# zer0int/OpenVision

Measured on AMD Instinct MI355X. Metric: images/sec (node) ViT-L/14@224 fwd+InfoNCE, higher is better.
Workload: dtype bf16; 1 GPU; vit-large-patch14-224: image tower + text tower (T=80) + InfoNCE, per-GPU batch 256, formula weights, bf16 MFMA / fp32 accumulate; fp8_mask=0, global_batch=256, micro_batches=1, parallelism=dp1

## Files before the change

openvision_amd/csrc/attention.hip:

```cpp
#include "common.h"
#include <stdlib.h>

namespace {

struct AttnArgs {
    const ov_bf16* qkv; int64_t ldq;
    ov_bf16* out; int64_t ldo;
    int B, L, H, nqt, KC;
    float scale_log2;
    int prefix;
};

typedef __attribute__((address_space(3))) s16x4_t* lds_s16x4_ptr;
typedef const __attribute__((address_space(1))) void* gptr_t;
typedef __attribute__((address_space(3))) void* lptr_t;

__device__ __forceinline__ bf16x8_t tr_pair(const char* p0, const char* p1) {
    const s16x4_t a = __builtin_amdgcn_ds_read_tr16_b64_v4i16((lds_s16x4_ptr)p0);
    const s16x4_t b = __builtin_amdgcn_ds_read_tr16_b64_v4i16((lds_s16x4_ptr)p1);
    typedef short s16x8_t __attribute__((ext_vector_type(8)));
    const s16x8_t c = {a[0], a[1], a[2], a[3], b[0], b[1], b[2], b[3]};
    return __builtin_bit_cast(bf16x8_t, c);
}

__device__ __forceinline__ u32x2_t tr_read_asm(const char* p) {
    u32x2_t v;
    const unsigned addr = (unsigned)(uintptr_t)(__attribute__((address_space(3))) const char*)p;
    asm volatile("ds_read_b64_tr_b16 %0, %1" : "=v"(v) : "v"(addr));
    return v;
}
__device__ __forceinline__ void tr_wait(u32x2_t (&t)[8]) {
    asm volatile("s_waitcnt lgkmcnt(0)"
                 : "+v"(t[0]), "+v"(t[1]), "+v"(t[2]), "+v"(t[3]), "+v"(t[4]), "+v"(t[5]), "+v"(t[6]), "+v"(t[7]));
}
__device__ __forceinline__ bf16x8_t tr_join(u32x2_t a, u32x2_t b) {
    const u32x4_t w = {a[0], a[1], b[0], b[1]};
    return __builtin_bit_cast(bf16x8_t, w);
}

__device__ __forceinline__ unsigned pack_fp8x4(float a, float b, float c, float d) {
    int w = 0;
    w = __builtin_amdgcn_cvt_pk_fp8_f32(__builtin_amdgcn_fmed3f(a, -448.f, 448.f), __builtin_amdgcn_fmed3f(b, -448.f, 448.f), w, false);
    w = __builtin_amdgcn_cvt_pk_fp8_f32(__builtin_amdgcn_fmed3f(c, -448.f, 448.f), __builtin_amdgcn_fmed3f(d, -448.f, 448.f), w, true);
    return (unsigned)w;
}

struct AttnPArgs {
    const ov_bf16* qkv; int64_t ldq;
    ov_bf16* out; int64_t ldo;
    int L, H, nqt, KC, nheads;
    float scale_log2;
    const float* out_amax;
    float* amax_next;
    int lone_valu;
    float* lse;
};

__device__ __forceinline__ void stage_head(const AttnPArgs& a, int bh, char* slot, int wave, int lane, int nthreads) {
    const int b = bh / a.H, h = bh - b * a.H;
    const int HD = a.H * 64, KC = a.KC, L = a.L;
    const char* base = (const char*)(a.qkv + (int64_t)b * L * a.ldq + h * 64);
    const unsigned rowb = (unsigned)(a.ldq * 2);
    const unsigned last = (unsigned)(L - 1) * rowb;
    char* ks = slot;
    char* vs = slot + KC * 128;
    const int nchunk = KC * 8;
    for (int q0c = wave * 64; q0c < nchunk; q0c += nthreads) {
        {
            const int kkey = (q0c + lane) >> 3;
            const unsigned ro = kkey < L ? (unsigned)kkey * rowb : last;
            const int c = (lane & 7) ^ ((kkey >> 1) & 7);
            __builtin_amdgcn_global_load_lds((gptr_t)(base + (ro + (unsigned)((HD + c * 8) * 2))), (lptr_t)(ks + q0c * 16), 16, 0, 0);
        }
        {
            const int dh = q0c >= KC * 4 ? 1 : 0;
            const int vkey = (q0c - dh * KC * 4 + lane) >> 2;
            const unsigned ro = vkey < L ? (unsigned)vkey * rowb : last;
            __builtin_amdgcn_global_load_lds((gptr_t)(base + (ro + (unsigned)((2 * HD + (dh * 4 + (lane & 3)) * 8) * 2))),
                                             (lptr_t)(vs + q0c * 16), 16, 0, 0);
        }
    }
}

__device__ __forceinline__ float max3_asm(float x, float y, float z) {
    float d;
    asm("v_max3_f32 %0, %1, %2, %3" : "=v"(d) : "v"(x), "v"(y), "v"(z));
    return d;
}
typedef float f32x2_t __attribute__((ext_vector_type(2)));
__device__ __forceinline__ void exp_rows(f32x16_t& s, float c, float nm, f32x2_t& acc) {
    const f32x2_t cc = {c, c}, mm = {nm, nm};
#pragma unroll
    for (int i = 0; i < 8; ++i) {
        f32x2_t v = {s[2 * i], s[2 * i + 1]};
        v = __builtin_elementwise_fma(v, cc, mm);
        v[0] = __builtin_amdgcn_exp2f(v[0]);
        v[1] = __builtin_amdgcn_exp2f(v[1]);
        acc += v;
        s[2 * i] = v[0];
        s[2 * i + 1] = v[1];
    }
}
template <int OFF>
__device__ __forceinline__ u32x2_t tr_read_off(unsigned addr) {
    u32x2_t v;
    asm volatile("ds_read_b64_tr_b16 %0, %1 offset:%2" : "=v"(v) : "v"(addr), "n"(OFF));
    return v;
}

template <bool DEEP, bool OUT8, bool LSE = false>
__global__ __launch_bounds__(DEEP ? 512 : 640, DEEP ? 2 : 3) void attn_fwd_hd64_persist(const AttnPArgs a) {
    extern __shared__ __attribute__((aligned(16))) char smem[];
    const int tid = threadIdx.x;
    const int lane = tid & 63;
    const int wave = __builtin_amdgcn_readfirstlane(tid >> 6);
    const int r = lane & 31, h2 = lane >> 5;
    const int L = a.L, KC = a.KC;
    const int slot_bytes = KC * 256;
    const int nk_tiles = (L + 31) >> 5;
    const bool lone_on = a.lone_valu != 0;
    const bool lone_key = lone_on && (L & 31) == 1 && (nk_tiles & 1) && nk_tiles > 1;
    const int n = (a.nheads - (int)blockIdx.x + (int)gridDim.x - 1) / (int)gridDim.x;
    if (n <= 0) return;
    const float inv8 = OUT8 ? __uint_as_float(__builtin_amdgcn_readfirstlane(__float_as_uint(448.0f / (2.0f * fmaxf(*a.out_amax, 1e-30f))))) : 1.0f;
    const float next_thr = (OUT8 && a.amax_next != nullptr)
                               ? __uint_as_float(__builtin_amdgcn_readfirstlane(__float_as_uint(*a.amax_next))) : 0.f;

    const int kb = r * 128 + ((h2 ^ ((r >> 1) & 7)) << 4);
    const int vi = lane & 15, vg = (lane >> 4) & 1;
    const int v_lane0 = KC * 128 + (4 * h2 + (vi >> 2)) * 64 + (16 * vg + 4 * (vi & 3)) * 2;
    const int v_lane1 = v_lane0 + KC * 64;
    const int q0 = wave * 32;
    int qrow = q0 + r;
    qrow = qrow < L ? qrow : L - 1;

    auto head_base = [&](int bh) {
        const int b = bh / a.H, h = bh - b * a.H;
        return a.qkv + (int64_t)b * L * a.ldq + h * 64;
    };
    auto row_offset = [&](int ld, int per_h2, unsigned bytes) {
        unsigned lf = (unsigned)lane;
        asm volatile("" : "+v"(lf));
        int qr = q0 + (int)(lf & 31u);
        qr = qr < L ? qr : L - 1;
        return (unsigned)(qr * ld + per_h2 * (int)(lf >> 5)) * bytes;
    };
    auto load_q = [&](u32x4_t (&q)[4], int bh) {
        const ov_bf16* qb = head_base(bh);
        const unsigned qoff = row_offset((int)a.ldq, 8, 2u);
        asm volatile("global_load_dwordx4 %0, %1, %2" : "=v"(q[0]) : "v"(qoff), "s"(qb) : "memory");
        asm volatile("global_load_dwordx4 %0, %1, %2 offset:32" : "=v"(q[1]) : "v"(qoff), "s"(qb) : "memory");
        asm volatile("global_load_dwordx4 %0, %1, %2 offset:64" : "=v"(q[2]) : "v"(qoff), "s"(qb) : "memory");
        asm volatile("global_load_dwordx4 %0, %1, %2 offset:96" : "=v"(q[3]) : "v"(qoff), "s"(qb) : "memory");
    };
    stage_head(a, blockIdx.x, smem, wave, lane, blockDim.x);
    u32x4_t qn[4];
    load_q(qn, blockIdx.x);
    asm volatile("s_waitcnt vmcnt(0)" : "+v"(qn[0]), "+v"(qn[1]), "+v"(qn[2]), "+v"(qn[3]) :: "memory");

    for (int j = 0; j < n; ++j) {
        const int bh = blockIdx.x + j * gridDim.x;
        bf16x8_t qf[4];
#pragma unroll
        for (int st = 0; st < 4; ++st) qf[st] = __builtin_bit_cast(bf16x8_t, qn[st]);
        asm volatile("s_barrier" ::: "memory");
        if (j + 1 < n) stage_head(a, bh + gridDim.x, smem + ((j + 1) & 1) * slot_bytes, wave, lane, blockDim.x);
        const char* ks = smem + (j & 1) * slot_bytes;
        const unsigned ks_u = (unsigned)(uintptr_t)(__attribute__((address_space(3))) const char*)ks;

        float m = -INFINITY, lsum = 0.f;
        f32x16_t o0, o1;
#pragma unroll
        for (int i = 0; i < 16; ++i) { o0[i] = 0.f; o1[i] = 0.f; }
        bf16x8_t kfa[4], kfb[4];
        auto load_k = [&](bf16x8_t (&kf)[4], int kt) {
            const unsigned kp = (unsigned)(kt * 4096 + kb);
#pragma unroll
            for (int st = 0; st < 4; ++st) kf[st] = *(const bf16x8_t*)(ks + (kp ^ (unsigned)(st * 32)));
        };
        auto mask_tail = [&](f32x16_t& sc, int kt) {
            if (kt * 32 + 32 > L) {
#pragma unroll
                for (int i = 0; i < 16; ++i) {
                    const int key = kt * 32 + (i & 3) + 8 * (i >> 2) + 4 * h2;
                    if (key >= L) sc[i] = -INFINITY;
                }
            }
        };
        auto tile_max = [&](const f32x16_t& sc) {
            float mx = max3_asm(max3_asm(sc[0], sc[1], sc[2]), max3_asm(sc[3], sc[4], sc[5]), max3_asm(sc[6], sc[7], sc[8]));
            return max3_asm(mx, max3_asm(sc[9], sc[10], sc[11]), max3_asm(max3_asm(sc[12], sc[13], sc[14]), sc[15], sc[15]));
        };
        auto pack_p = [&](const f32x16_t& sc, int st) {
            const u32x4_t w = {pack_bf16x2(sc[8 * st + 0], sc[8 * st + 1]), pack_bf16x2(sc[8 * st + 2], sc[8 * st + 3]),
                               pack_bf16x2(sc[8 * st + 4], sc[8 * st + 5]), pack_bf16x2(sc[8 * st + 6], sc[8 * st + 7])};
            return __builtin_bit_cast(bf16x8_t, w);
        };
        const int npair = nk_tiles >> 1;
        load_k(kfa, 0);
        if (DEEP && npair > 0) load_k(kfb, 1);
        for (int it = 0; it < npair; ++it) {
            const int kt = 2 * it;
            const unsigned va0 = ks_u + kt * 2048 + v_lane0, va1 = ks_u + kt * 2048 + v_lane1;
            if (!DEEP) load_k(kfb, kt + 1);
            u32x2_t vt[8], vu[8];
            auto read_vt = [&]() {
                vt[0] = tr_read_off<0>(va0);    vt[1] = tr_read_off<512>(va0);
                vt[2] = tr_read_off<0>(va1);    vt[3] = tr_read_off<512>(va1);
                vt[4] = tr_read_off<1024>(va0); vt[5] = tr_read_off<1536>(va0);
                vt[6] = tr_read_off<1024>(va1); vt[7] = tr_read_off<1536>(va1);
            };
            if (DEEP) read_vt();
            if (DEEP) {
                vu[0] = tr_read_off<2048>(va0); vu[1] = tr_read_off<2560>(va0);
                vu[2] = tr_read_off<2048>(va1); vu[3] = tr_read_off<2560>(va1);
                vu[4] = tr_read_off<3072>(va0); vu[5] = tr_read_off<3584>(va0);
                vu[6] = tr_read_off<3072>(va1); vu[7] = tr_read_off<3584>(va1);
            }
            f32x16_t sa, sb;
#pragma unroll
            for (int i = 0; i < 16; ++i) { sa[i] = 0.f; sb[i] = 0.f; }
#pragma unroll
            for (int st = 0; st < 4; ++st) sa = __builtin_amdgcn_mfma_f32_32x32x16_bf16(kfa[st], qf[st], sa, 0, 0, 0);
#pragma unroll
            for (int st = 0; st < 4; ++st) sb = __builtin_amdgcn_mfma_f32_32x32x16_bf16(kfb[st], qf[st], sb, 0, 0, 0);
            if (!DEEP) read_vt();
            if (kt + 2 < nk_tiles) load_k(kfa, kt + 2);
            else if (DEEP) asm volatile("s_nop 7" : "+v"(sb));
            if (DEEP && kt + 3 < nk_tiles) load_k(kfb, kt + 3);
            mask_tail(sb, kt + 1);
            float mx = fmaxf(tile_max(sa), tile_max(sb));
            {
                const auto sw = __builtin_amdgcn_permlane32_swap(__float_as_uint(mx), __float_as_uint(mx), false, false);
                mx = fmaxf(__uint_as_float(sw[0]), __uint_as_float(sw[1])) * a.scale_log2;
            }
            if (!__all(mx - m <= 8.0f)) {
                const float mn = fmaxf(m, mx);
                const float alpha = __builtin_amdgcn_exp2f(m - mn);
                m = mn;
                lsum *= alpha;
#pragma unroll
                for (int i = 0; i < 16; ++i) { o0[i] *= alpha; o1[i] *= alpha; }
            }
            const float nm = -m;
            f32x2_t ps = {0.f, 0.f};
            exp_rows(sa, a.scale_log2, nm, ps);
            exp_rows(sb, a.scale_log2, nm, ps);
            lsum += ps[0] + ps[1];
            const bf16x8_t pa0 = pack_p(sa, 0), pa1 = pack_p(sa, 1), pb0 = pack_p(sb, 0), pb1 = pack_p(sb, 1);
            tr_wait(vt);
            __builtin_amdgcn_sched_barrier(0);
            if (!DEEP) {
                vu[0] = tr_read_off<2048>(va0); vu[1] = tr_read_off<2560>(va0);
                vu[2] = tr_read_off<2048>(va1); vu[3] = tr_read_off<2560>(va1);
                vu[4] = tr_read_off<3072>(va0); vu[5] = tr_read_off<3584>(va0);
                vu[6] = tr_read_off<3072>(va1); vu[7] = tr_read_off<3584>(va1);
            }
            o0 = __builtin_amdgcn_mfma_f32_32x32x16_bf16(tr_join(vt[0], vt[1]), pa0, o0, 0, 0, 0);
            o1 = __builtin_amdgcn_mfma_f32_32x32x16_bf16(tr_join(vt[2], vt[3]), pa0, o1, 0, 0, 0);
            o0 = __builtin_amdgcn_mfma_f32_32x32x16_bf16(tr_join(vt[4], vt[5]), pa1, o0, 0, 0, 0);
            o1 = __builtin_amdgcn_mfma_f32_32x32x16_bf16(tr_join(vt[6], vt[7]), pa1, o1, 0, 0, 0);
            tr_wait(vu);
            __builtin_amdgcn_sched_barrier(0);
            o0 = __builtin_amdgcn_mfma_f32_32x32x16_bf16(tr_join(vu[0], vu[1]), pb0, o0, 0, 0, 0);
            o1 = __builtin_amdgcn_mfma_f32_32x32x16_bf16(tr_join(vu[2], vu[3]), pb0, o1, 0, 0, 0);
            o0 = __builtin_amdgcn_mfma_f32_32x32x16_bf16(tr_join(vu[4], vu[5]), pb1, o0, 0, 0, 0);
            o1 = __builtin_amdgcn_mfma_f32_32x32x16_bf16(tr_join(vu[6], vu[7]), pb1, o1, 0, 0, 0);
        }
        if (j + 1 < n) load_q(qn, bh + gridDim.x);
        if (lone_key) {
            float s0 = 0.f, s1 = 0.f;
#pragma unroll
            for (int st = 0; st < 4; ++st) {
                const u32x4_t kq = __builtin_bit_cast(u32x4_t, kfa[st]), qq = __builtin_bit_cast(u32x4_t, qf[st]);
                asm("v_dot2c_f32_bf16 %0, %1, %2" : "+v"(s0) : "v"(qq[0]), "v"(kq[0]));
                asm("v_dot2c_f32_bf16 %0, %1, %2" : "+v"(s1) : "v"(qq[1]), "v"(kq[1]));
                asm("v_dot2c_f32_bf16 %0, %1, %2" : "+v"(s0) : "v"(qq[2]), "v"(kq[2]));
                asm("v_dot2c_f32_bf16 %0, %1, %2" : "+v"(s1) : "v"(qq[3]), "v"(kq[3]));
            }
            asm("s_nop 2" : "+v"(s0), "+v"(s1));
            float sd = s0 + s1;
            {
                const auto sw = __builtin_amdgcn_permlane32_swap(__float_as_uint(sd), __float_as_uint(sd), false, false);
                sd = __uint_as_float(sw[0]) + __uint_as_float(sw[1]);
            }
            const char* vrow = ks + KC * 128 + (L - 1) * 64 + 8 * h2;
            u32x2_t v0[4];
#pragma unroll
            for (int g = 0; g < 4; ++g) v0[g] = *(const u32x2_t*)(vrow + g * 16);
            const float mx = sd * a.scale_log2;
            if (!__all(mx - m <= 8.0f)) {
                const float mn = fmaxf(m, mx);
                const float alpha = __builtin_amdgcn_exp2f(m - mn);
                m = mn;
                lsum *= alpha;
#pragma unroll
                for (int i = 0; i < 16; ++i) { o0[i] *= alpha; o1[i] *= alpha; }
            }
            const float pk = __builtin_amdgcn_exp2f(mx - m);
            lsum += h2 ? 0.f : pk;
#pragma unroll
            for (int g = 0; g < 4; ++g) {
                o0[4 * g + 0] = fmaf(pk, bf16lo_to_f32(v0[g][0]), o0[4 * g + 0]);
                o0[4 * g + 1] = fmaf(pk, bf16hi_to_f32(v0[g][0]), o0[4 * g + 1]);
                o0[4 * g + 2] = fmaf(pk, bf16lo_to_f32(v0[g][1]), o0[4 * g + 2]);
                o0[4 * g + 3] = fmaf(pk, bf16hi_to_f32(v0[g][1]), o0[4 * g + 3]);
            }
            __builtin_amdgcn_sched_barrier(0);
#pragma unroll
            for (int g = 0; g < 4; ++g) v0[g] = *(const u32x2_t*)(vrow + KC * 64 + g * 16);
#pragma unroll
            for (int g = 0; g < 4; ++g) {
                o1[4 * g + 0] = fmaf(pk, bf16lo_to_f32(v0[g][0]), o1[4 * g + 0]);
                o1[4 * g + 1] = fmaf(pk, bf16hi_to_f32(v0[g][0]), o1[4 * g + 1]);
                o1[4 * g + 2] = fmaf(pk, bf16lo_to_f32(v0[g][1]), o1[4 * g + 2]);
                o1[4 * g + 3] = fmaf(pk, bf16hi_to_f32(v0[g][1]), o1[4 * g + 3]);
            }
        } else if (nk_tiles & 1) {
            const int kt = nk_tiles - 1;
            unsigned lf = (unsigned)lane;
            asm volatile("" : "+v"(lf));
            const unsigned vif = lf & 15u, vgf = (lf >> 4) & 1u, h2f = lf >> 5;
            const unsigned vl0 = (unsigned)KC * 128u + (4u * h2f + (vif >> 2)) * 64u + (16u * vgf + 4u * (vif & 3u)) * 2u;
            const unsigned va0 = ks_u + kt * 2048 + vl0, va1 = va0 + (unsigned)KC * 64u;
            u32x2_t vt[8];
            vt[0] = tr_read_off<0>(va0);    vt[1] = tr_read_off<512>(va0);
            vt[2] = tr_read_off<0>(va1);    vt[3] = tr_read_off<512>(va1);
            vt[4] = tr_read_off<1024>(va0); vt[5] = tr_read_off<1536>(va0);
            vt[6] = tr_read_off<1024>(va1); vt[7] = tr_read_off<1536>(va1);
            f32x16_t sa;
#pragma unroll
            for (int i = 0; i < 16; ++i) sa[i] = 0.f;
#pragma unroll
            for (int st = 0; st < 4; ++st) sa = __builtin_amdgcn_mfma_f32_32x32x16_bf16(kfa[st], qf[st], sa, 0, 0, 0);
            mask_tail(sa, kt);
            asm volatile("s_nop 15" : "+v"(sa));
            float mx = tile_max(sa);
            {
                const auto sw = __builtin_amdgcn_permlane32_swap(__float_as_uint(mx), __float_as_uint(mx), false, false);
                mx = fmaxf(__uint_as_float(sw[0]), __uint_as_float(sw[1])) * a.scale_log2;
            }
            if (!__all(mx - m <= 8.0f)) {
                const float mn = fmaxf(m, mx);
                const float alpha = __builtin_amdgcn_exp2f(m - mn);
                m = mn;
                lsum *= alpha;
#pragma unroll
                for (int i = 0; i < 16; ++i) { o0[i] *= alpha; o1[i] *= alpha; }
            }
            const float nm = -m;
            f32x2_t ps = {0.f, 0.f};
            exp_rows(sa, a.scale_log2, nm, ps);
            lsum += ps[0] + ps[1];
            const bf16x8_t pa0 = pack_p(sa, 0), pa1 = pack_p(sa, 1);
            tr_wait(vt);
            __builtin_amdgcn_sched_barrier(0);
            o0 = __builtin_amdgcn_mfma_f32_32x32x16_bf16(tr_join(vt[0], vt[1]), pa0, o0, 0, 0, 0);
            o1 = __builtin_amdgcn_mfma_f32_32x32x16_bf16(tr_join(vt[2], vt[3]), pa0, o1, 0, 0, 0);
            o0 = __builtin_amdgcn_mfma_f32_32x32x16_bf16(tr_join(vt[4], vt[5]), pa1, o0, 0, 0, 0);
            o1 = __builtin_amdgcn_mfma_f32_32x32x16_bf16(tr_join(vt[6], vt[7]), pa1, o1, 0, 0, 0);
        }
        float l;
        {
            const auto sw = __builtin_amdgcn_permlane32_swap(__float_as_uint(lsum), __float_as_uint(lsum), false, false);
            l = __uint_as_float(sw[0]) + __uint_as_float(sw[1]);
        }
        float inv = 1.0f / l;
        if (OUT8) {
            if (a.amax_next != nullptr) {
                float lm = 0.f;
#pragma unroll
                for (int i = 0; i < 16; ++i) lm = fmaxf(lm, fmaxf(fabsf(o0[i]), fabsf(o1[i])));
                lm *= inv;
#pragma unroll
                for (int o = 32; o > 0; o >>= 1) lm = fmaxf(lm, __shfl_xor(lm, o, 64));
                if (lane == 0 && lm > next_thr) atomicMax((unsigned*)a.amax_next, __float_as_uint(lm));
            }
            inv *= inv8;
            const unsigned char* ob = (const unsigned char*)a.out + (int64_t)(bh / a.H) * L * a.ldo + (bh % a.H) * 64;
            const unsigned ooff = row_offset((int)a.ldo, 4, 1u);
#define OV_ST8(GQ)                                                                                                         \
            {                                                                                                              \
                const unsigned w0 = pack_fp8x4(o0[4 * GQ] * inv, o0[4 * GQ + 1] * inv, o0[4 * GQ + 2] * inv, o0[4 * GQ + 3] * inv); \
                const unsigned w1 = pack_fp8x4(o1[4 * GQ] * inv, o1[4 * GQ + 1] * inv, o1[4 * GQ + 2] * inv, o1[4 * GQ + 3] * inv); \
                asm volatile("global_store_dword %0, %1, %2 offset:%3" :: "v"(ooff), "v"(w0), "s"(ob), "n"(8 * GQ) : "memory");        \
                asm volatile("global_store_dword %0, %1, %2 offset:%3\n\ts_nop 0" :: "v"(ooff), "v"(w1), "s"(ob), "n"(32 + 8 * GQ) : "memory"); \
            }
            OV_ST8(0) OV_ST8(1) OV_ST8(2) OV_ST8(3)
#undef OV_ST8
        } else {
            const ov_bf16* ob = a.out + (int64_t)(bh / a.H) * L * a.ldo + (bh % a.H) * 64;
            const unsigned ooff = row_offset((int)a.ldo, 8, 2u);
#define OV_ST16(O, P, BYTE_OFF)                                                                                              \
            {                                                                                                               \
                const unsigned ax = pack_bf16x2(O[8 * P + 0] * inv, O[8 * P + 1] * inv), ay = pack_bf16x2(O[8 * P + 2] * inv, O[8 * P + 3] * inv); \
                const unsigned bx = pack_bf16x2(O[8 * P + 4] * inv, O[8 * P + 5] * inv), by = pack_bf16x2(O[8 * P + 6] * inv, O[8 * P + 7] * inv); \
                const auto sx = __builtin_amdgcn_permlane32_swap(ax, bx, false, false);                                       \
                const auto sy = __builtin_amdgcn_permlane32_swap(ay, by, false, false);                                       \
                const u32x4_t w = {sx[0], sy[0], sx[1], sy[1]};                                                               \
                 \
                                                      \
                asm volatile("global_store_dwordx4 %0, %1, %2 offset:%3\n\ts_nop 1" :: "v"(ooff), "v"(w), "s"(ob), "n"(BYTE_OFF) : "memory"); \
            }
            OV_ST16(o0, 0, 0) OV_ST16(o0, 1, 32) OV_ST16(o1, 0, 64) OV_ST16(o1, 1, 96)
#undef OV_ST16
        }
        if (LSE && !OUT8) {
            const float v = m + __builtin_amdgcn_logf(l);
            const float* lb = a.lse + (int64_t)bh * KC;
            const unsigned loff = row_offset(1, 0, 4u);
            asm volatile("global_store_dword %0, %1, %2" :: "v"(loff), "v"(v), "s"(lb) : "memory");
        }
        if (OUT8) asm volatile("s_waitcnt vmcnt(8)" : "+v"(qn[0]), "+v"(qn[1]), "+v"(qn[2]), "+v"(qn[3]) :: "memory");
        else if (LSE) asm volatile("s_waitcnt vmcnt(5)" : "+v"(qn[0]), "+v"(qn[1]), "+v"(qn[2]), "+v"(qn[3]) :: "memory");
        else asm volatile("s_waitcnt vmcnt(4)" : "+v"(qn[0]), "+v"(qn[1]), "+v"(qn[2]), "+v"(qn[3]) :: "memory");
    }
}

struct AttnSArgs {
    const ov_bf16* qkv; int64_t ldq;
    ov_bf16* out; int64_t ldo;
    int L, H, nqt, nqb, nheads, nchunks;
    float scale_log2;
    const float* out_amax;
    float* amax_next;
    int lone_valu;
};

template <bool OUT8>
__global__ __launch_bounds__(512, 4) void attn_fwd_hd64_stream(const AttnSArgs a) {
    extern __shared__ __attribute__((aligned(16))) char smem[];
    const int tid = threadIdx.x;
    const int lane = tid & 63;
    const int wave = __builtin_amdgcn_readfirstlane(tid >> 6);
    const int r = lane & 31, h2 = lane >> 5;
    const int L = a.L;
    const int wid = blockIdx.x;
    const int xcd = wid & 7, slot_id = wid >> 3;
    const int bh = (slot_id / a.nqb) * 8 + xcd, qb = slot_id % a.nqb;
    if (bh >= a.nheads) return;
    const int b = bh / a.H, h = bh - b * a.H;
    const int HD = a.H * 64;
    const ov_bf16* base = a.qkv + (int64_t)b * L * a.ldq + h * 64;
    const int qt = qb * 8 + wave;
    const bool active = qt < a.nqt;
    int qrow = qt * 32 + r;
    qrow = qrow < L ? qrow : L - 1;

    char* const sdst = smem + wave * 1024;
    const int nc = a.nchunks;
    const char* const bbase = (const char*)base;
    unsigned kofs = (unsigned)(((tid >> 3) * a.ldq + HD + (((tid & 7) ^ ((tid >> 4) & 7)) * 8)) * 2);
    unsigned vofs = (unsigned)(((((tid & 255) >> 2)) * a.ldq + 2 * HD + ((tid >> 8) * 4 + (tid & 3)) * 8) * 2);
    const unsigned cstep = (unsigned)(64 * a.ldq * 2);
    auto stage = [&](int c) {
        char* dst = sdst + (c & 3) * 16384;
        unsigned ko = kofs, vo = vofs;
        if (c == nc - 1) {
            const int t = threadIdx.x;
            const int over_k = c * 64 + (t >> 3) - (L - 1), over_v = c * 64 + ((t & 255) >> 2) - (L - 1);
            if (over_k > 0) ko -= (unsigned)(over_k * a.ldq * 2);
            if (over_v > 0) vo -= (unsigned)(over_v * a.ldq * 2);
        }
        __builtin_amdgcn_global_load_lds((gptr_t)(bbase + ko), (lptr_t)dst, 16, 0, 0);
        __builtin_amdgcn_global_load_lds((gptr_t)(bbase + vo), (lptr_t)(dst + 8192), 16, 0, 0);
        kofs += cstep;
        vofs += cstep;
    };
    bf16x8_t qf[4];
// ... 111 lines not shown
        const char* ks = smem + ((nc - 1) & 3) * 16384;
        float s0 = 0.f, s1 = 0.f;
#pragma unroll
        for (int st = 0; st < 4; ++st) {
            const u32x4_t kq = *(const u32x4_t*)(ks + (2 * st + h2) * 16), qq = __builtin_bit_cast(u32x4_t, qf[st]);
            asm("v_dot2c_f32_bf16 %0, %1, %2" : "+v"(s0) : "v"(qq[0]), "v"(kq[0]));
            asm("v_dot2c_f32_bf16 %0, %1, %2" : "+v"(s1) : "v"(qq[1]), "v"(kq[1]));
            asm("v_dot2c_f32_bf16 %0, %1, %2" : "+v"(s0) : "v"(qq[2]), "v"(kq[2]));
            asm("v_dot2c_f32_bf16 %0, %1, %2" : "+v"(s1) : "v"(qq[3]), "v"(kq[3]));
        }
        asm("s_nop 2" : "+v"(s0), "+v"(s1));
        float sd = s0 + s1;
        {
            const auto sw = __builtin_amdgcn_permlane32_swap(__float_as_uint(sd), __float_as_uint(sd), false, false);
            sd = __uint_as_float(sw[0]) + __uint_as_float(sw[1]);
        }
        const float mx = sd * a.scale_log2;
        if (!__all(mx - m <= 8.0f)) {
            const float mn = fmaxf(m, mx);
            const float alpha = __builtin_amdgcn_exp2f(m - mn);
            m = mn;
            lsum *= alpha;
#pragma unroll
            for (int i = 0; i < 16; ++i) { o0[i] *= alpha; o1[i] *= alpha; }
        }
        const float pk = __builtin_amdgcn_exp2f(mx - m);
        lsum += h2 ? 0.f : pk;
        const char* vrow = ks + 8192 + 8 * h2;
#pragma unroll
        for (int g = 0; g < 4; ++g) {
            const u32x2_t v0 = *(const u32x2_t*)(vrow + g * 16), v1 = *(const u32x2_t*)(vrow + 4096 + g * 16);
            o0[4 * g + 0] = fmaf(pk, bf16lo_to_f32(v0[0]), o0[4 * g + 0]);
            o0[4 * g + 1] = fmaf(pk, bf16hi_to_f32(v0[0]), o0[4 * g + 1]);
            o0[4 * g + 2] = fmaf(pk, bf16lo_to_f32(v0[1]), o0[4 * g + 2]);
            o0[4 * g + 3] = fmaf(pk, bf16hi_to_f32(v0[1]), o0[4 * g + 3]);
            o1[4 * g + 0] = fmaf(pk, bf16lo_to_f32(v1[0]), o1[4 * g + 0]);
            o1[4 * g + 1] = fmaf(pk, bf16hi_to_f32(v1[0]), o1[4 * g + 1]);
            o1[4 * g + 2] = fmaf(pk, bf16lo_to_f32(v1[1]), o1[4 * g + 2]);
            o1[4 * g + 3] = fmaf(pk, bf16hi_to_f32(v1[1]), o1[4 * g + 3]);
        }
    }
    float l;
    {
        const auto sw = __builtin_amdgcn_permlane32_swap(__float_as_uint(lsum), __float_as_uint(lsum), false, false);
        l = __uint_as_float(sw[0]) + __uint_as_float(sw[1]);
    }
    float inv = 1.0f / l;
    if (OUT8 && a.amax_next != nullptr) {
        float lm = 0.f;
#pragma unroll
        for (int i = 0; i < 16; ++i) lm = fmaxf(lm, fmaxf(fabsf(o0[i]), fabsf(o1[i])));
        lm = qt * 32 + r < L ? lm * inv : 0.f;
#pragma unroll
        for (int o = 32; o > 0; o >>= 1) lm = fmaxf(lm, __shfl_xor(lm, o, 64));
        if (lane == 0 && lm > *(volatile float*)a.amax_next) atomicMax((unsigned*)a.amax_next, __float_as_uint(lm));
    }
    if (qt * 32 + r < L) {
        if (OUT8) {
            inv *= 448.0f / (2.0f * fmaxf(*a.out_amax, 1e-30f));
            unsigned char* op = (unsigned char*)a.out + ((int64_t)b * L + qrow) * a.ldo + h * 64 + 4 * h2;
#pragma unroll
            for (int gq = 0; gq < 4; ++gq) {
                *(unsigned*)(op + 8 * gq) = pack_fp8x4(o0[4 * gq] * inv, o0[4 * gq + 1] * inv, o0[4 * gq + 2] * inv, o0[4 * gq + 3] * inv);
                *(unsigned*)(op + 32 + 8 * gq) = pack_fp8x4(o1[4 * gq] * inv, o1[4 * gq + 1] * inv, o1[4 * gq + 2] * inv, o1[4 * gq + 3] * inv);
            }
        } else {
            ov_bf16* op = a.out + ((int64_t)b * L + qrow) * a.ldo + h * 64 + 4 * h2;
#pragma unroll
            for (int gq = 0; gq < 4; ++gq) {
                const u32x2_t w0 = {pack_bf16x2(o0[4 * gq] * inv, o0[4 * gq + 1] * inv),
                                    pack_bf16x2(o0[4 * gq + 2] * inv, o0[4 * gq + 3] * inv)};
                const u32x2_t w1 = {pack_bf16x2(o1[4 * gq] * inv, o1[4 * gq + 1] * inv),
                                    pack_bf16x2(o1[4 * gq + 2] * inv, o1[4 * gq + 3] * inv)};
                *(u32x2_t*)(op + 8 * gq) = w0;
                *(u32x2_t*)(op + 32 + 8 * gq) = w1;
            }
        }
    }
}

template <int HDP, bool MASK = false>
__global__ __launch_bounds__(640) void attn_fwd_generic(const AttnArgs a, int hd) {
    constexpr bool SWZ = HDP == 64;
    constexpr int KS = HDP / 16;
    constexpr int DT = HDP / 32;
    constexpr int CH = HDP / 8;
    extern __shared__ __attribute__((aligned(16))) char smem[];
    const int tid = threadIdx.x, nthreads = blockDim.x;
    const int lane = tid & 63, wave = tid >> 6, nw = nthreads >> 6;
    const int r = lane & 31, h2 = lane >> 5;
    const int bh = blockIdx.x, b = bh / a.H, h = bh - b * a.H;
    const int L = a.L, KC = a.KC;
    const int HD = a.H * hd;
    char* ks = smem;
    char* vs = smem + KC * HDP * 2;
    const ov_bf16* base = a.qkv + (int64_t)b * L * a.ldq + h * hd;
    const int qt = blockIdx.y * nw + wave;
    const bool active = qt < a.nqt;
    const int q0 = qt * 32;

    bf16x8_t qf[KS];
    {
        int qrow = q0 + r;
        qrow = (active && qrow < L) ? qrow : L - 1;
        const ov_bf16* qp = base + (int64_t)qrow * a.ldq;
#pragma unroll
        for (int s = 0; s < KS; ++s) {
            const int d = 16 * s + 8 * h2;
            u32x4_t w = {0u, 0u, 0u, 0u};
            if (d < hd) w = *(const u32x4_t*)(qp + d);
            qf[s] = __builtin_bit_cast(bf16x8_t, w);
        }
    }
    float m = -INFINITY, lsum = 0.f;
    f32x16_t o[DT];
#pragma unroll
    for (int t = 0; t < DT; ++t)
#pragma unroll
        for (int i = 0; i < 16; ++i) o[t][i] = 0.f;
    const int vi = lane & 15, vg = (lane >> 4) & 1;
    const int v_lane_off = (4 * h2 + (vi >> 2)) * 64 + (16 * vg + 4 * (vi & 3)) * 2;

    const int kend_wg = MASK ? min(L, max(a.prefix, min(a.nqt, ((int)blockIdx.y + 1) * nw) * 32)) : L;
    const int kvis = MASK ? min(L, max(a.prefix, q0 + 32)) : L;
    for (int kc0 = 0; kc0 < kend_wg; kc0 += KC) {
        if (kc0) __syncthreads();
        for (int idx = tid; idx < KC * CH; idx += nthreads) {
            const int row = idx / CH, c = idx - row * CH;
            u32x4_t kv = {0u, 0u, 0u, 0u}, vv = {0u, 0u, 0u, 0u};
            if (kc0 + row < L && c * 8 < hd) {
                const ov_bf16* p = base + (int64_t)(kc0 + row) * a.ldq + HD + c * 8;
                kv = *(const u32x4_t*)p;
                vv = *(const u32x4_t*)(p + HD);
            }
            *(u32x4_t*)(ks + row * (HDP * 2) + ((SWZ ? c ^ ((row >> 1) & 7) : c) << 4)) = kv;
            *(u32x4_t*)(vs + (c >> 2) * (KC * 64) + row * 64 + (c & 3) * 16) = vv;
        }
        __syncthreads();
        if (!active || kvis <= kc0) continue;
        const int nk = (kvis - kc0) < KC ? (kvis - kc0) : KC;
        const bool lone_key = (nk & 31) == 1 && nk > 32;
        const int ntile = ((nk + 31) >> 5) - (lone_key ? 1 : 0);
        for (int kt = 0; kt < ntile; ++kt) {
            f32x16_t s;
#pragma unroll
            for (int i = 0; i < 16; ++i) s[i] = 0.f;
            const char* kp = ks + (kt * 32 + r) * (HDP * 2);
#pragma unroll
            for (int st = 0; st < KS; ++st) {
                const int c = 2 * st + h2;
                const bf16x8_t kf = *(const bf16x8_t*)(kp + ((SWZ ? c ^ ((r >> 1) & 7) : c) << 4));
                s = __builtin_amdgcn_mfma_f32_32x32x16_bf16(kf, qf[st], s, 0, 0, 0);
            }
            if (kt * 32 + 32 > nk) {
#pragma unroll
                for (int i = 0; i < 16; ++i) {
                    const int key = kt * 32 + (i & 3) + 8 * (i >> 2) + 4 * h2;
                    if (key >= nk) s[i] = -INFINITY;
                }
            }
            if (MASK && kc0 + kt * 32 + 31 >= a.prefix && kc0 + kt * 32 + 31 > q0) {
#pragma unroll
                for (int i = 0; i < 16; ++i) {
                    const int key = kc0 + kt * 32 + (i & 3) + 8 * (i >> 2) + 4 * h2;
                    if (key >= a.prefix && key > q0 + r) s[i] = -INFINITY;
                }
            }
            asm volatile("s_nop 15" : "+v"(s));
            float mx = max3_asm(max3_asm(s[0], s[1], s[2]), max3_asm(s[3], s[4], s[5]), max3_asm(s[6], s[7], s[8]));
            mx = max3_asm(mx, max3_asm(s[9], s[10], s[11]), max3_asm(max3_asm(s[12], s[13], s[14]), s[15], s[15]));
            {
                const auto sw = __builtin_amdgcn_permlane32_swap(__float_as_uint(mx), __float_as_uint(mx), false, false);
                mx = fmaxf(__uint_as_float(sw[0]), __uint_as_float(sw[1])) * a.scale_log2;
            }
            if (MASK ? __any(mx - m > 8.0f) : !__all(mx - m <= 8.0f)) {
                const float mn = (!MASK || mx - m > 8.0f) ? fmaxf(m, mx) : m;
                const float alpha = __builtin_amdgcn_exp2f(m - mn);
                m = mn;
                lsum *= alpha;
#pragma unroll
                for (int t = 0; t < DT; ++t)
#pragma unroll
                    for (int i = 0; i < 16; ++i) o[t][i] *= alpha;
            }
            const float nm = -m;
            f32x2_t ps = {0.f, 0.f};
            exp_rows(s, a.scale_log2, nm, ps);
            lsum += ps[0] + ps[1];
            bf16x8_t pf[2];
#pragma unroll
            for (int st = 0; st < 2; ++st) {
                u32x4_t w = {pack_bf16x2(s[8 * st + 0], s[8 * st + 1]), pack_bf16x2(s[8 * st + 2], s[8 * st + 3]),
                             pack_bf16x2(s[8 * st + 4], s[8 * st + 5]), pack_bf16x2(s[8 * st + 6], s[8 * st + 7])};
                pf[st] = __builtin_bit_cast(bf16x8_t, w);
            }
            const char* vp = vs + kt * 32 * 64 + v_lane_off;
#pragma unroll
            for (int st = 0; st < 2; ++st) {
#pragma unroll
                for (int t = 0; t < DT; ++t) {
                    const char* v0 = vp + t * (KC * 64) + st * 16 * 64;
                    o[t] = __builtin_amdgcn_mfma_f32_32x32x16_bf16(tr_pair(v0, v0 + 8 * 64), pf[st], o[t], 0, 0, 0);
                }
            }
        }
        if (lone_key) {
            const int key = nk - 1;
            const char* kp = ks + key * (HDP * 2);
            float s0 = 0.f, s1 = 0.f;
#pragma unroll
            for (int st = 0; st < KS; ++st) {
                const int c = 2 * st + h2;
                const u32x4_t kq = *(const u32x4_t*)(kp + ((SWZ ? c ^ ((key >> 1) & 7) : c) << 4)), qq = __builtin_bit_cast(u32x4_t, qf[st]);
                asm("v_dot2c_f32_bf16 %0, %1, %2" : "+v"(s0) : "v"(qq[0]), "v"(kq[0]));
                asm("v_dot2c_f32_bf16 %0, %1, %2" : "+v"(s1) : "v"(qq[1]), "v"(kq[1]));
                asm("v_dot2c_f32_bf16 %0, %1, %2" : "+v"(s0) : "v"(qq[2]), "v"(kq[2]));
                asm("v_dot2c_f32_bf16 %0, %1, %2" : "+v"(s1) : "v"(qq[3]), "v"(kq[3]));
            }
            asm("s_nop 2" : "+v"(s0), "+v"(s1));
            float sd = s0 + s1;
            {
                const auto sw = __builtin_amdgcn_permlane32_swap(__float_as_uint(sd), __float_as_uint(sd), false, false);
                sd = __uint_as_float(sw[0]) + __uint_as_float(sw[1]);
            }
            const bool seen = !MASK || kc0 + key < a.prefix || kc0 + key <= q0 + r;
            const float mx = seen ? sd * a.scale_log2 : -INFINITY;
            if (MASK ? __any(mx - m > 8.0f) : !__all(mx - m <= 8.0f)) {
                const float mn = (!MASK || mx - m > 8.0f) ? fmaxf(m, mx) : m;
                const float alpha = __builtin_amdgcn_exp2f(m - mn);
                m = mn;
                lsum *= alpha;
#pragma unroll
                for (int t = 0; t < DT; ++t)
#pragma unroll
                    for (int i = 0; i < 16; ++i) o[t][i] *= alpha;
            }
            const float pk = __builtin_amdgcn_exp2f(mx - m);
            lsum += h2 ? 0.f : pk;
#pragma unroll
            for (int t = 0; t < DT; ++t) {
                const char* vrow = vs + t * (KC * 64) + key * 64 + 8 * h2;
#pragma unroll
                for (int g = 0; g < 4; ++g) {
                    const u32x2_t v = *(const u32x2_t*)(vrow + g * 16);
                    o[t][4 * g + 0] = fmaf(pk, bf16lo_to_f32(v[0]), o[t][4 * g + 0]);
                    o[t][4 * g + 1] = fmaf(pk, bf16hi_to_f32(v[0]), o[t][4 * g + 1]);
                    o[t][4 * g + 2] = fmaf(pk, bf16lo_to_f32(v[1]), o[t][4 * g + 2]);
                    o[t][4 * g + 3] = fmaf(pk, bf16hi_to_f32(v[1]), o[t][4 * g + 3]);
                }
            }
        }
    }
    if (!active) return;
    const float l = lsum + __shfl_xor(lsum, 32, 64);
    const float inv = 1.0f / l;
    const int q = q0 + r;
    if (q < L) {
        ov_bf16* op = a.out + ((int64_t)b * L + q) * a.ldo + h * hd + 4 * h2;
#pragma unroll
        for (int t = 0; t < DT; ++t)
#pragma unroll
            for (int g = 0; g < 4; ++g) {
                const int d = t * 32 + 8 * g + 4 * h2;
                if (d < hd) {
                    const u32x2_t w = {pack_bf16x2(o[t][4 * g] * inv, o[t][4 * g + 1] * inv),
                                       pack_bf16x2(o[t][4 * g + 2] * inv, o[t][4 * g + 3] * inv)};
                    *(u32x2_t*)(op + t * 32 + 8 * g) = w;
                }
            }
    }
}

}

namespace {
int attention_impl(const ov_bf16* qkv, int64_t ld_qkv, ov_bf16* out, int64_t ld_out, int B, int L, int H, int hd, float scale,
                   const float* out_amax, float* amax_next, float* lse, ov_stream_t stream);
}

extern "C" int ov_attention(const ov_bf16* qkv, int64_t ld_qkv, ov_bf16* out, int64_t ld_out, int B, int L,
                            int H, int hd, float scale, ov_stream_t stream) {
    return attention_impl(qkv, ld_qkv, out, ld_out, B, L, H, hd, scale, nullptr, nullptr, nullptr, stream);
}

extern "C" int ov_attention_lse(const ov_bf16* qkv, int64_t ld_qkv, ov_bf16* out, int64_t ld_out, float* lse, int B, int L, int H, int hd,
                                float scale, ov_stream_t stream) {
    if (!lse || ((uintptr_t)lse & 3)) return OV_ERR_INVALID;
    return attention_impl(qkv, ld_qkv, out, ld_out, B, L, H, hd, scale, nullptr, nullptr, lse, stream);
}

extern "C" int ov_attention_fp8out(const ov_bf16* qkv, int64_t ld_qkv, unsigned char* out8, int64_t ld_out, int B, int L, int H,
                                   int hd, float scale, const float* out_amax, float* out_amax_next, ov_stream_t stream) {
    if (!out_amax) return OV_ERR_INVALID;
    if (hd != 64) return OV_ERR_UNSUPPORTED;
    return attention_impl(qkv, ld_qkv, (ov_bf16*)out8, ld_out, B, L, H, hd, scale, out_amax, out_amax_next, nullptr, stream);
}

namespace {
int attn_lone_valu() {
    static const int v = [] { const char* e = getenv("OVHIP_ATTN_LONEKEY"); return (e && e[0] == '0') ? 0 : 1; }();
    return v;
}

int attention_impl(const ov_bf16* qkv, int64_t ld_qkv, ov_bf16* out, int64_t ld_out, int B, int L, int H, int hd, float scale,
                   const float* out_amax, float* amax_next, float* lse, ov_stream_t stream) {
    if (!qkv || !out || B <= 0 || L <= 0 || H <= 0) return OV_ERR_INVALID;
    if (hd <= 0 || hd % 8 || hd > 96) return OV_ERR_UNSUPPORTED;
    if (ld_qkv % 8 || ld_out % 8 || ld_qkv < 3 * H * hd || ld_out < H * hd) return OV_ERR_INVALID;
    if (((uintptr_t)qkv | (uintptr_t)out) & 15) return OV_ERR_INVALID;
    const bool out8 = out_amax != nullptr;
    if (lse != nullptr && (!ov_attn_bwd_resident(hd, L) || out8)) return OV_ERR_UNSUPPORTED;
    const int nqt = (L + 31) / 32, lp = nqt * 32;
    const float scale_log2 = scale * 1.4426950408889634f;
    const bool narrow = (int64_t)L * ld_qkv * 2 < 0x7fffffffLL && (int64_t)L * ld_out * 2 < 0x7fffffffLL;
    if (hd == 64 && lp <= 320 && narrow) {
        AttnPArgs p;
        p.qkv = qkv; p.ldq = ld_qkv; p.out = out; p.ldo = ld_out;
        p.L = L; p.H = H; p.nqt = nqt; p.KC = lp; p.nheads = B * H; p.scale_log2 = scale_log2; p.out_amax = out_amax; p.amax_next = amax_next; p.lse = lse;
        p.lone_valu = attn_lone_valu();
        static OvPerDeviceOnce attr2;
        const int dev_attr2 = ov_current_device();
        if (attr2.need(dev_attr2)) {
            hipError_t e = hipFuncSetAttribute((const void*)attn_fwd_hd64_persist<false, false>, hipFuncAttributeMaxDynamicSharedMemorySize,
                                               160 * 1024);
            if (e == hipSuccess)
                e = hipFuncSetAttribute((const void*)attn_fwd_hd64_persist<true, false>, hipFuncAttributeMaxDynamicSharedMemorySize, 160 * 1024);
            if (e == hipSuccess)
                e = hipFuncSetAttribute((const void*)attn_fwd_hd64_persist<false, true>, hipFuncAttributeMaxDynamicSharedMemorySize, 160 * 1024);
            if (e == hipSuccess)
                e = hipFuncSetAttribute((const void*)attn_fwd_hd64_persist<true, true>, hipFuncAttributeMaxDynamicSharedMemorySize, 160 * 1024);
            if (e == hipSuccess)
                e = hipFuncSetAttribute((const void*)attn_fwd_hd64_persist<false, false, true>, hipFuncAttributeMaxDynamicSharedMemorySize, 160 * 1024);
            if (e == hipSuccess)
                e = hipFuncSetAttribute((const void*)attn_fwd_hd64_persist<true, false, true>, hipFuncAttributeMaxDynamicSharedMemorySize, 160 * 1024);
            if (e != hipSuccess) return OV_ERR_HIP - (int)e;
            attr2.mark(dev_attr2);
        }
        const int ncu = ov_num_cus();
        const size_t smem = (size_t)2 * lp * 256;
        int per_cu = (int)((160 * 1024) / smem);
        const int by_waves = (nqt <= 8 ? 8 : 12) / nqt;
        if (per_cu > by_waves) per_cu = by_waves;
        if (per_cu < 1) per_cu = 1;
        const int cap = ncu * per_cu;
        const int grid = p.nheads < cap ? p.nheads : cap;
        const dim3 pg((unsigned)grid), pb(nqt * 64);
        if (nqt <= 8) {
            if (out8) hipLaunchKernelGGL((attn_fwd_hd64_persist<true, true>), pg, pb, smem, (hipStream_t)stream, p);
            else if (lse) hipLaunchKernelGGL((attn_fwd_hd64_persist<true, false, true>), pg, pb, smem, (hipStream_t)stream, p);
            else hipLaunchKernelGGL((attn_fwd_hd64_persist<true, false>), pg, pb, smem, (hipStream_t)stream, p);
        } else {
            if (out8) hipLaunchKernelGGL((attn_fwd_hd64_persist<false, true>), pg, pb, smem, (hipStream_t)stream, p);
            else if (lse) hipLaunchKernelGGL((attn_fwd_hd64_persist<false, false, true>), pg, pb, smem, (hipStream_t)stream, p);
            else hipLaunchKernelGGL((attn_fwd_hd64_persist<false, false>), pg, pb, smem, (hipStream_t)stream, p);
        }
        OV_LAUNCH_CHECK();
        return OV_OK;
    }
    if (hd == 64 && lp > 320) {
        AttnSArgs sa;
        sa.qkv = qkv; sa.ldq = ld_qkv; sa.out = out; sa.ldo = ld_out;
        sa.L = L; sa.H = H; sa.nqt = nqt; sa.nqb = (nqt + 7) / 8; sa.nheads = B * H; sa.nchunks = (L + 63) / 64;
        sa.scale_log2 = scale_log2;
        sa.out_amax = out_amax;
        sa.amax_next = amax_next;
        sa.lone_valu = attn_lone_valu();
        static OvPerDeviceOnce attr4;
        const int dev_attr4 = ov_current_device();
        if (attr4.need(dev_attr4)) {
            hipError_t e = hipFuncSetAttribute((const void*)attn_fwd_hd64_stream<false>, hipFuncAttributeMaxDynamicSharedMemorySize, 160 * 1024);
            if (e == hipSuccess)
                e = hipFuncSetAttribute((const void*)attn_fwd_hd64_stream<true>, hipFuncAttributeMaxDynamicSharedMemorySize, 160 * 1024);
            if (e != hipSuccess) return OV_ERR_HIP - (int)e;
            attr4.mark(dev_attr4);
        }
        const int64_t heads8 = ((int64_t)sa.nheads + 7) / 8 * 8;
        const int64_t nwg = heads8 * sa.nqb;
        if (nwg > 0x7fffffffLL) return OV_ERR_UNSUPPORTED;
        if (out8) hipLaunchKernelGGL(attn_fwd_hd64_stream<true>, dim3((unsigned)nwg), dim3(512), 4 * 16384, (hipStream_t)stream, sa);
        else hipLaunchKernelGGL(attn_fwd_hd64_stream<false>, dim3((unsigned)nwg), dim3(512), 4 * 16384, (hipStream_t)stream, sa);
        OV_LAUNCH_CHECK();
        return OV_OK;
    }
    if (lse != nullptr || out8) return OV_ERR_UNSUPPORTED;
    AttnArgs g;
    g.qkv = qkv; g.ldq = ld_qkv; g.out = out; g.ldo = ld_out;
    g.B = B; g.L = L; g.H = H; g.nqt = nqt;
    g.scale_log2 = scale_log2;
    g.prefix = L;
    const bool resident = lp <= 320;
    g.KC = resident ? lp : 256;
    const int nwg = resident ? g.nqt : 8;
    const size_t smem = (size_t)g.KC * 96 * 4;
    static OvPerDeviceOnce attr3;
    const int dev_attr3 = ov_current_device();
    if (attr3.need(dev_attr3)) {
        hipError_t e = hipFuncSetAttribute((const void*)attn_fwd_generic<96>, hipFuncAttributeMaxDynamicSharedMemorySize,
                                           160 * 1024);
        if (e != hipSuccess) return OV_ERR_HIP - (int)e;
        attr3.mark(dev_attr3);
    }
    hipLaunchKernelGGL(attn_fwd_generic<96>, dim3((unsigned)(B * H), (unsigned)((g.nqt + nwg - 1) / nwg)), dim3(nwg * 64), smem,
                       (hipStream_t)stream, g, hd);
    OV_LAUNCH_CHECK();
    return OV_OK;
}
}

extern "C" int ov_attention_prefix(const ov_bf16* qkv, int64_t ld_qkv, ov_bf16* out, int64_t ld_out, int B, int L, int H, int hd, float scale,
                                   int prefix, ov_stream_t stream) {
    if (!qkv || !out || B <= 0 || L <= 0 || H <= 0) return OV_ERR_INVALID;
    if (prefix < 0 || prefix > L) return OV_ERR_INVALID;
    if (prefix == L) return ov_attention(qkv, ld_qkv, out, ld_out, B, L, H, hd, scale, stream);
    if (hd <= 0 || hd % 8 || hd > 96) return OV_ERR_UNSUPPORTED;
    if (ld_qkv % 8 || ld_out % 8 || ld_qkv < 3 * H * hd || ld_out < H * hd) return OV_ERR_INVALID;
    if (((uintptr_t)qkv | (uintptr_t)out) & 15) return OV_ERR_INVALID;
    if ((int64_t)B * H > 0x7fffffffLL) return OV_ERR_UNSUPPORTED;
    AttnArgs g;
    g.qkv = qkv; g.ldq = ld_qkv; g.out = out; g.ldo = ld_out;
    g.B = B; g.L = L; g.H = H; g.nqt = (L + 31) / 32;
    g.scale_log2 = scale * 1.4426950408889634f;
    g.prefix = prefix;
    const int lp = g.nqt * 32;
    const bool resident = lp <= 320;
    g.KC = resident ? lp : 256;
    const int nwg = resident ? g.nqt : 8;
    const int hdp = hd == 64 ? 64 : 96;
    const size_t smem = (size_t)g.KC * hdp * 4;
    static OvPerDeviceOnce attr;
    const int dev = ov_current_device();
    if (attr.need(dev)) {
        hipError_t e = hipFuncSetAttribute((const void*)attn_fwd_generic<64, true>, hipFuncAttributeMaxDynamicSharedMemorySize, 160 * 1024);
        if (e == hipSuccess)
            e = hipFuncSetAttribute((const void*)attn_fwd_generic<96, true>, hipFuncAttributeMaxDynamicSharedMemorySize, 160 * 1024);
        if (e != hipSuccess) return OV_ERR_HIP - (int)e;
        attr.mark(dev);
    }
    const dim3 grid((unsigned)(B * H), (unsigned)((g.nqt + nwg - 1) / nwg)), blk(nwg * 64);
    if (hdp == 64) hipLaunchKernelGGL((attn_fwd_generic<64, true>), grid, blk, smem, (hipStream_t)stream, g, hd);
    else hipLaunchKernelGGL((attn_fwd_generic<96, true>), grid, blk, smem, (hipStream_t)stream, g, hd);
    OV_LAUNCH_CHECK();
    return OV_OK;
}
```

Before: 5818 images/sec.

## Add dedicated producer wave to stage K/V tiles in persistent attention

For certain query-tile counts, the persistent hd64 attention kernel now launches one extra wave that only stages the next head's K/V into the double-buffered LDS slot. It runs at raised priority and keeps in step with the compute waves through barriers. Previously every compute wave shared the staging work between heads. The goal is to take global-load issue off the compute waves so loads overlap with MFMA work better. In exchange, each block carries an extra wave that can reduce occupancy, the launch-bounds and by-waves math changes, and the non-deep path is now always instantiated with the stager.

New measurement: 5843 images/sec (median of 6 runs). Within noise of the previous version (+0.4%).

```diff
diff --git a/openvision_amd/csrc/attention.hip b/openvision_amd/csrc/attention.hip
--- a/openvision_amd/csrc/attention.hip
+++ b/openvision_amd/csrc/attention.hip
@@ -108,20 +108,33 @@
     return v;
 }
 
-template <bool DEEP, bool OUT8, bool LSE = false>
-__global__ __launch_bounds__(DEEP ? 512 : 640, DEEP ? 2 : 3) void attn_fwd_hd64_persist(const AttnPArgs a) {
+template <bool DEEP, bool OUT8, bool LSE, bool STAGER>
+__global__ __launch_bounds__(DEEP ? 512 : 768, DEEP ? 2 : 3) void attn_fwd_hd64_persist(const AttnPArgs a) {
     extern __shared__ __attribute__((aligned(16))) char smem[];
     const int tid = threadIdx.x;
     const int lane = tid & 63;
     const int wave = __builtin_amdgcn_readfirstlane(tid >> 6);
     const int r = lane & 31, h2 = lane >> 5;
     const int L = a.L, KC = a.KC;
-    const int slot_bytes = KC * 256;
     const int nk_tiles = (L + 31) >> 5;
     const bool lone_on = a.lone_valu != 0;
     const bool lone_key = lone_on && (L & 31) == 1 && (nk_tiles & 1) && nk_tiles > 1;
     const int n = (a.nheads - (int)blockIdx.x + (int)gridDim.x - 1) / (int)gridDim.x;
     if (n <= 0) return;
+    const int slot_bytes = KC * 256;
+    if (STAGER && wave == a.nqt) {
+        asm volatile("s_setprio 3");
+        stage_head(a, blockIdx.x, smem, 0, lane, 64);
+        asm volatile("s_waitcnt vmcnt(0)" ::: "memory");
+        for (int j = 0; j < n; ++j) {
+            asm volatile("s_barrier" ::: "memory");
+            if (j + 1 < n) {
+                stage_head(a, blockIdx.x + (j + 1) * gridDim.x, smem + ((j + 1) & 1) * slot_bytes, 0, lane, 64);
+                asm volatile("s_waitcnt vmcnt(0)" ::: "memory");
+            }
+        }
+        return;
+    }
     const float inv8 = OUT8 ? __uint_as_float(__builtin_amdgcn_readfirstlane(__float_as_uint(448.0f / (2.0f * fmaxf(*a.out_amax, 1e-30f))))) : 1.0f;
     const float next_thr = (OUT8 && a.amax_next != nullptr)
                                ? __uint_as_float(__builtin_amdgcn_readfirstlane(__float_as_uint(*a.amax_next))) : 0.f;
@@ -153,7 +166,7 @@
         asm volatile("global_load_dwordx4 %0, %1, %2 offset:64" : "=v"(q[2]) : "v"(qoff), "s"(qb) : "memory");
         asm volatile("global_load_dwordx4 %0, %1, %2 offset:96" : "=v"(q[3]) : "v"(qoff), "s"(qb) : "memory");
     };
-    stage_head(a, blockIdx.x, smem, wave, lane, blockDim.x);
+    if (!STAGER) stage_head(a, blockIdx.x, smem, wave, lane, blockDim.x);
     u32x4_t qn[4];
     load_q(qn, blockIdx.x);
     asm volatile("s_waitcnt vmcnt(0)" : "+v"(qn[0]), "+v"(qn[1]), "+v"(qn[2]), "+v"(qn[3]) :: "memory");
@@ -164,7 +177,7 @@
 #pragma unroll
         for (int st = 0; st < 4; ++st) qf[st] = __builtin_bit_cast(bf16x8_t, qn[st]);
         asm volatile("s_barrier" ::: "memory");
-        if (j + 1 < n) stage_head(a, bh + gridDim.x, smem + ((j + 1) & 1) * slot_bytes, wave, lane, blockDim.x);
+        if (!STAGER && j + 1 < n) stage_head(a, bh + gridDim.x, smem + ((j + 1) & 1) * slot_bytes, wave, lane, blockDim.x);
         const char* ks = smem + (j & 1) * slot_bytes;
         const unsigned ks_u = (unsigned)(uintptr_t)(__attribute__((address_space(3))) const char*)ks;
 
@@ -882,6 +895,25 @@
     return v;
 }
 
+bool attn_stager(int nqt) { return nqt == 3 || (nqt >= 5 && nqt <= 7) || nqt >= 9; }
+
+template <bool DEEP, bool STAGER>
+hipError_t persist_lds_attr() {
+    hipError_t e = hipFuncSetAttribute((const void*)attn_fwd_hd64_persist<DEEP, false, false, STAGER>, hipFuncAttributeMaxDynamicSharedMemorySize,
+                                       160 * 1024);
+    if (e == hipSuccess)
+        e = hipFuncSetAttribute((const void*)attn_fwd_hd64_persist<DEEP, true, false, STAGER>, hipFuncAttributeMaxDynamicSharedMemorySize, 160 * 1024);
+    if (e == hipSuccess)
+        e = hipFuncSetAttribute((const void*)attn_fwd_hd64_persist<DEEP, false, true, STAGER>, hipFuncAttributeMaxDynamicSharedMemorySize, 160 * 1024);
+    return e;
+}
+template <bool DEEP, bool STAGER>
+void persist_launch(bool out8, bool lse, dim3 pg, dim3 pb, size_t smem, hipStream_t stream, const AttnPArgs& p) {
+    if (out8) hipLaunchKernelGGL((attn_fwd_hd64_persist<DEEP, true, false, STAGER>), pg, pb, smem, stream, p);
+    else if (lse) hipLaunchKernelGGL((attn_fwd_hd64_persist<DEEP, false, true, STAGER>), pg, pb, smem, stream, p);
+    else hipLaunchKernelGGL((attn_fwd_hd64_persist<DEEP, false, false, STAGER>), pg, pb, smem, stream, p);
+}
+
 int attention_impl(const ov_bf16* qkv, int64_t ld_qkv, ov_bf16* out, int64_t ld_out, int B, int L, int H, int hd, float scale,
                    const float* out_amax, float* amax_next, float* lse, ov_stream_t stream) {
     if (!qkv || !out || B <= 0 || L <= 0 || H <= 0) return OV_ERR_INVALID;
@@ -898,42 +930,30 @@
         p.qkv = qkv; p.ldq = ld_qkv; p.out = out; p.ldo = ld_out;
         p.L = L; p.H = H; p.nqt = nqt; p.KC = lp; p.nheads = B * H; p.scale_log2 = scale_log2; p.out_amax = out_amax; p.amax_next = amax_next; p.lse = lse;
         p.lone_valu = attn_lone_valu();
+        const bool stager = attn_stager(nqt);
         static OvPerDeviceOnce attr2;
         const int dev_attr2 = ov_current_device();
         if (attr2.need(dev_attr2)) {
-            hipError_t e = hipFuncSetAttribute((const void*)attn_fwd_hd64_persist<false, false>, hipFuncAttributeMaxDynamicSharedMemorySize,
-                                               160 * 1024);
-            if (e == hipSuccess)
-                e = hipFuncSetAttribute((const void*)attn_fwd_hd64_persist<true, false>, hipFuncAttributeMaxDynamicSharedMemorySize, 160 * 1024);
-            if (e == hipSuccess)
-                e = hipFuncSetAttribute((const void*)attn_fwd_hd64_persist<false, true>, hipFuncAttributeMaxDynamicSharedMemorySize, 160 * 1024);
-            if (e == hipSuccess)
-                e = hipFuncSetAttribute((const void*)attn_fwd_hd64_persist<true, true>, hipFuncAttributeMaxDynamicSharedMemorySize, 160 * 1024);
-            if (e == hipSuccess)
-                e = hipFuncSetAttribute((const void*)attn_fwd_hd64_persist<false, false, true>, hipFuncAttributeMaxDynamicSharedMemorySize, 160 * 1024);
-            if (e == hipSuccess)
-                e = hipFuncSetAttribute((const void*)attn_fwd_hd64_persist<true, false, true>, hipFuncAttributeMaxDynamicSharedMemorySize, 160 * 1024);
+            hipError_t e = persist_lds_attr<true, false>();
+            if (e == hipSuccess) e = persist_lds_attr<true, true>();
+            if (e == hipSuccess) e = persist_lds_attr<false, true>();
             if (e != hipSuccess) return OV_ERR_HIP - (int)e;
             attr2.mark(dev_attr2);
         }
         const int ncu = ov_num_cus();
         const size_t smem = (size_t)2 * lp * 256;
         int per_cu = (int)((160 * 1024) / smem);
-        const int by_waves = (nqt <= 8 ? 8 : 12) / nqt;
+        const int nw = nqt + (stager ? 1 : 0);
+        const bool deep = nw <= 8;
+        const int by_waves = (deep ? 8 : 12) / nw;
         if (per_cu > by_waves) per_cu = by_waves;
         if (per_cu < 1) per_cu = 1;
         const int cap = ncu * per_cu;
         const int grid = p.nheads < cap ? p.nheads : cap;
-        const dim3 pg((unsigned)grid), pb(nqt * 64);
-        if (nqt <= 8) {
-            if (out8) hipLaunchKernelGGL((attn_fwd_hd64_persist<true, true>), pg, pb, smem, (hipStream_t)stream, p);
-            else if (lse) hipLaunchKernelGGL((attn_fwd_hd64_persist<true, false, true>), pg, pb, smem, (hipStream_t)stream, p);
-            else hipLaunchKernelGGL((attn_fwd_hd64_persist<true, false>), pg, pb, smem, (hipStream_t)stream, p);
-        } else {
-            if (out8) hipLaunchKernelGGL((attn_fwd_hd64_persist<false, true>), pg, pb, smem, (hipStream_t)stream, p);
-            else if (lse) hipLaunchKernelGGL((attn_fwd_hd64_persist<false, false, true>), pg, pb, smem, (hipStream_t)stream, p);
-            else hipLaunchKernelGGL((attn_fwd_hd64_persist<false, false>), pg, pb, smem, (hipStream_t)stream, p);
-        }
+        const dim3 pg((unsigned)grid), pb(nw * 64);
+        if (deep && stager) persist_launch<true, true>(out8, lse != nullptr, pg, pb, smem, (hipStream_t)stream, p);
+        else if (deep) persist_launch<true, false>(out8, lse != nullptr, pg, pb, smem, (hipStream_t)stream, p);
+        else persist_launch<false, true>(out8, lse != nullptr, pg, pb, smem, (hipStream_t)stream, p);
         OV_LAUNCH_CHECK();
         return OV_OK;
     }
```
